# mlvlab/UP-NeRF

Measured on AMD Instinct MI355X. Metric: training rays/sec, higher is better.
Workload: dtype f32 (f16x3 emulated: 3 fp16 MFMAs per product, fp32 accumulate); 1 GPU; BASELINE.json configs[1]: Brandenburg Gate shape, 4096 rays/GPU/step, 64 coarse + 128 fine samples, two 8x256 fields + candidate/colour heads + TransientNet + appearance/candidate embeddings (763 images), pose optimisation ON, full step incl. both Adam updates; rays_per_gpu=4096, n_images=763, N_samples=64, N_importance=128, parallelism=dp1, field=f16x3

## Files before the change

upnerf_amd/csrc/common.cuh:

```cuda
#pragma once
#include <hip/hip_runtime.h>
#include <stdint.h>
#include "upnerf_hip.h"

typedef float f32x16 __attribute__((ext_vector_type(16)));
typedef float f32x4 __attribute__((ext_vector_type(4)));

#define NTHREADS 256

#define HIP_TRY(expr)                        \
  do {                                       \
    hipError_t _e = (expr);                  \
    if (_e != hipSuccess) return (int)_e;    \
  } while (0)

__device__ __forceinline__ int swz(int row, int k, int ldw) {
  return row * ldw + ((((k >> 2) ^ (row & 15)) << 2) | (k & 3));
}
__device__ __forceinline__ int swz4(int row, int k, int ldw) { return row * ldw + (((k >> 2) ^ (row & 15)) << 2); }

__device__ __forceinline__ float softplus_f(float x) { return x > 20.0f ? x : log1pf(expf(x)); }
__device__ __forceinline__ float sigmoid_f(float x) { return 1.0f / (1.0f + expf(-x)); }

__device__ __forceinline__ double wave_sum_f64(double v) {
// ... 155 lines not shown
      }
    }
  return ((unsigned long long)hi << 32) | lo;
}

template <int MT, int NT>
__device__ __forceinline__ void acc_apply_mask(f32x16 (&acc)[MT][NT], unsigned long long bits) {
  const unsigned int lo = (unsigned int)bits, hi = (unsigned int)(bits >> 32);
#pragma unroll
  for (int mt = 0; mt < MT; ++mt)
#pragma unroll
    for (int nt = 0; nt < NT; ++nt)
#pragma unroll
      for (int r = 0; r < 16; ++r) {
        const int e = (mt * NT + nt) * 16 + r;
        const bool on = e < 32 ? (lo >> e) & 1u : (hi >> (e - 32)) & 1u;
        acc[mt][nt][r] = on ? acc[mt][nt][r] : 0.0f;
      }
}

template <int MT, int NT>
__device__ __forceinline__ void acc_track_max(const f32x16 (&acc)[MT][NT], float* __restrict__ slot, int lane) {
  if (!slot) return;
  float m = 0.0f;
#pragma unroll
  for (int mt = 0; mt < MT; ++mt)
#pragma unroll
    for (int nt = 0; nt < NT; ++nt)
#pragma unroll
      for (int r = 0; r < 16; ++r) m = fmaxf(m, fabsf(acc[mt][nt][r]));
#pragma unroll
  for (int d = 32; d >= 1; d >>= 1) m = fmaxf(m, __shfl_xor(m, d));
  if (lane == 0) atomicMax((unsigned int*)slot, __float_as_uint(m));
}
__device__ __forceinline__ void wave_track_max(float m, float* __restrict__ slot, int lane) {
  if (!slot) return;
#pragma unroll
  for (int d = 32; d >= 1; d >>= 1) m = fmaxf(m, __shfl_xor(m, d));
  if (lane == 0) atomicMax((unsigned int*)slot, __float_as_uint(m));
}

template <int MT, int NT>
__device__ __forceinline__ void acc_to_lds(const f32x16 (&acc)[MT][NT], float* Hs, int ldw, int row0, int n0, int c0,
                                           int lane) {
  const int i = lane & 31, hh = lane >> 5;
#pragma unroll
  for (int mt = 0; mt < MT; ++mt)
#pragma unroll
    for (int nt = 0; nt < NT; ++nt)
#pragma unroll
      for (int r = 0; r < 16; ++r) {
        const int row = row0 + 32 * mt + (r & 3) + 8 * (r >> 2) + 4 * hh;
        Hs[swz(row, c0 + n0 + 32 * nt + i, ldw)] = acc[mt][nt][r];
      }
}

template <int TILE>
__device__ __forceinline__ void tile_store(const float* Hs, int ldw, int c0, int ncols, float* __restrict__ dst, int ldg,
                                           int m0, int M, int tid) {
  const int gpr = ncols >> 2;
  for (int idx = tid; idx < TILE * gpr; idx += NTHREADS) {
    const int row = idx / gpr, g = idx - row * gpr;
    if (m0 + row < M) {
      const f32x4 v = *(const f32x4*)&Hs[swz4(row, c0 + 4 * g, ldw)];
      *(f32x4*)&dst[(size_t)(m0 + row) * ldg + 4 * g] = v;
    }
  }
}

template <int TILE>
__device__ __forceinline__ void tile_mask_store(float* Hs, int ldw, int c0, int ncols, const float* __restrict__ act,
                                                float* __restrict__ gz, int ldg, int m0, int M, int tid) {
  const int gpr = ncols >> 2;
  for (int idx = tid; idx < TILE * gpr; idx += NTHREADS) {
    const int row = idx / gpr, g = idx - row * gpr;
    float* p = &Hs[swz4(row, c0 + 4 * g, ldw)];
    f32x4 v = {0.f, 0.f, 0.f, 0.f};
    if (m0 + row < M) {
      const size_t off = (size_t)(m0 + row) * ldg + 4 * g;
      const f32x4 av = *(const f32x4*)&act[off];
      v = *(const f32x4*)p;
      v.x = av.x > 0.f ? v.x : 0.f;
      v.y = av.y > 0.f ? v.y : 0.f;
      v.z = av.z > 0.f ? v.z : 0.f;
      v.w = av.w > 0.f ? v.w : 0.f;
      *(f32x4*)&gz[off] = v;
    }
    *(f32x4*)p = v;
  }
}

template <int TILE>
__device__ __forceinline__ void tile_rank1_store(float* Hs, int ldw, int ncols, const float* __restrict__ wrow,
                                                 const float* __restrict__ grow, int S, float* __restrict__ gz,
                                                 int m0, int M, int tid, float* __restrict__ maxslot = nullptr) {
  const int gpr = ncols >> 2;
  float lmax = 0.0f;
  for (int idx = tid; idx < TILE * gpr; idx += NTHREADS) {
    const int row = idx / gpr, g = idx - row * gpr, m = m0 + row;
    float* p = &Hs[swz4(row, 4 * g, ldw)];
    f32x4 v = {0.f, 0.f, 0.f, 0.f};
    if (m < M) {
      v = *(const f32x4*)p;
      if (grow) {
        const float w = wrow[m];
        const f32x4 gv = *(const f32x4*)&grow[(size_t)(m / S) * ncols + 4 * g];
        v.x += w * gv.x; v.y += w * gv.y; v.z += w * gv.z; v.w += w * gv.w;
      }
      *(f32x4*)&gz[(size_t)m * ncols + 4 * g] = v;
    }
    *(f32x4*)p = v;
    lmax = fmaxf(lmax, fmaxf(fmaxf(fabsf(v.x), fabsf(v.y)), fmaxf(fabsf(v.z), fabsf(v.w))));
  }
  wave_track_max(lmax, maxslot, tid & 63);
}

#define PI_F 3.14159274101257324f

__device__ __forceinline__ float mul_then_add(float o, float d, float z) {
#pragma clang fp contract(off)
  const float p = d * z;
  return o + p;
}

__device__ __forceinline__ void sincos_f32_via_f64(float arg, float& sn, float& cs) {
  const double x = (double)arg;
  const double q = rint(x * 0.63661977236758134308);
  double r = fma(-q, 1.57079632679489655800e+00, x);
  r = fma(-q, 6.12323399573676603587e-17, r);
  const double z = r * r;
  const double ps = -1.66666666666666324348e-01 + z * (8.33333333332248946124e-03 + z * (-1.98412698298579493134e-04 +
                    z * (2.75573137070700676789e-06 + z * (-2.50507602534068634195e-08 + z * 1.58969099521155010221e-10))));
  const double pc = 4.16666666666666019037e-02 + z * (-1.38888888888741095749e-03 + z * (2.48015872894767294178e-05 +
                    z * (-2.75573143513906633035e-07 + z * (2.08757232129817482790e-09 + z * -1.13596475577881948265e-11))));
  const double s = r + r * z * ps;
  const double c = 1.0 - 0.5 * z + z * z * pc;
  const int n = (int)(long long)q & 3;
  const double so = (n & 1) ? c : s, co = (n & 1) ? s : c;
  sn = (float)((n & 2) ? -so : so);
  cs = (float)(((n + 1) & 2) ? -co : co);
}

__device__ __forceinline__ float wave_sum(float v) {
#pragma unroll
  for (int d = 32; d >= 1; d >>= 1) v += __shfl_xor(v, d);
  return v;
}

#define NT_LOAD(p) __builtin_nontemporal_load(p)
#define NT_STORE(p, v) __builtin_nontemporal_store((v), (p))

#define RED_RG 8
#define RED_THREADS (64 * RED_RG)
template <int PW = RED_RG>
__device__ __forceinline__ void wgrad_reduce_body(int bid, int tid, const upnerf_wgrad_pending& P, f32x4 (*part)[64]) {
  static_assert(PW == 8 || PW == 4, "8 thread groups on 8 or 4 waves");
  const int N = P.N, K = P.K, TN = P.TN, TK = P.TK, nsplit = P.nsplit;
  const float* __restrict__ slabs = P.slabs;
  const float* __restrict__ bslabs = P.bslabs;
  const int lane = tid & 63;
  const int q = bid * 64 + lane;
  const int K4 = K >> 2;
  const int gy = (N + TN - 1) / TN, gz = (K + TK - 1) / TK;
  const bool ok = q < N * K4;
  const int n = ok ? q / K4 : 0, k = ok ? (q - n * K4) * 4 : 0;
  const int by = n / TN, bz = k / TK;
  const size_t off = ((size_t)by * gz + bz) * TN * TK + (size_t)(n - by * TN) * TK + (k - bz * TK);
  const size_t stride = (size_t)gy * gz * TN * TK;
#pragma unroll 1
  for (int rg = tid >> 6; rg < RED_RG; rg += PW) {
    f32x4 s[8];
#pragma unroll
    for (int u = 0; u < 8; ++u) s[u] = f32x4{0.f, 0.f, 0.f, 0.f};
    if (ok) {
      int sp = rg;
      for (; sp + 7 * RED_RG < nsplit; sp += 8 * RED_RG) {
        f32x4 v[8];
#pragma unroll
        for (int u = 0; u < 8; ++u) v[u] = *(const f32x4*)&slabs[off + (size_t)(sp + u * RED_RG) * stride];
#pragma unroll
        for (int u = 0; u < 8; ++u) s[u] += v[u];
      }
      for (; sp < nsplit; sp += RED_RG) s[0] += *(const f32x4*)&slabs[off + (size_t)sp * stride];
    }
    part[rg][lane] = ((s[0] + s[1]) + (s[2] + s[3])) + ((s[4] + s[5]) + (s[6] + s[7]));
  }
  __syncthreads();
  if ((tid >> 6) == 0 && ok) {
    const f32x4 t = ((part[0][lane] + part[1][lane]) + (part[2][lane] + part[3][lane])) +
                    ((part[4][lane] + part[5][lane]) + (part[6][lane] + part[7][lane]));
    if (P.n2 > 0 && n >= P.n2) *(f32x4*)&P.dW2[(size_t)(n - P.n2) * P.ldo2 + k] = t;
    else *(f32x4*)&P.dW[(size_t)n * P.ldo + k] = t;
  }
  if (P.db || (P.n2 > 0 && P.db2)) {
#pragma unroll 1
    for (int idx = bid * RED_THREADS + tid; idx < (bid + 1) * RED_THREADS; idx += 64 * PW)
    if (idx < N) {
      const int bby = idx / TN;
      float p[8] = {0.f, 0.f, 0.f, 0.f, 0.f, 0.f, 0.f, 0.f};
      const float* src = bslabs + (size_t)bby * TN + (idx - bby * TN);
      const size_t bst = (size_t)gy * TN;
      int sp = 0;
      for (; sp + 8 <= nsplit; sp += 8) {
#pragma unroll
        for (int u = 0; u < 8; ++u) p[u] += src[(size_t)(sp + u) * bst];
      }
      for (; sp < nsplit; ++sp) p[0] += src[(size_t)sp * bst];
      const float sb = ((p[0] + p[1]) + (p[2] + p[3])) + ((p[4] + p[5]) + (p[6] + p[7]));
      if (P.n2 > 0 && idx >= P.n2) { if (P.db2) P.db2[idx - P.n2] = sb; }
      else if (P.db) P.db[idx] = sb;
    }
  }
  if (P.vslabs && bid == 0) {
    for (int idx = tid; idx <= K; idx += 64 * PW) {
      float p[8] = {0.f, 0.f, 0.f, 0.f, 0.f, 0.f, 0.f, 0.f};
      const float* src = P.vslabs + idx;
      const size_t st = (size_t)K + 4;
      int sp = 0;
      for (; sp + 8 <= nsplit; sp += 8) {
#pragma unroll
        for (int u = 0; u < 8; ++u) p[u] += src[(size_t)(sp + u) * st];
      }
      for (; sp < nsplit; ++sp) p[0] += src[(size_t)sp * st];
      const float sv = ((p[0] + p[1]) + (p[2] + p[3])) + ((p[4] + p[5]) + (p[6] + p[7]));
      if (idx < K) P.dv[idx] = sv;
      else if (P.dbv) P.dbv[0] = sv;
    }
  }
}
```

upnerf_amd/csrc/wgrad_f16x3.hip:

```cpp
#include "common.cuh"
#include "wgrad_host.h"

namespace {

typedef _Float16 h8 __attribute__((ext_vector_type(8)));
typedef _Float16 h4 __attribute__((ext_vector_type(4)));
typedef short s4 __attribute__((ext_vector_type(4)));
typedef unsigned int u32x2_t __attribute__((ext_vector_type(2)));

#ifndef FX_CHUNK_BIG
#define FX_CHUNK_BIG 16
#endif

template <int FX_CHUNK>
__device__ __forceinline__ int himg(int row, int col) {
  const int panel = col >> 7, c = col & 127;
  return panel * (FX_CHUNK * 256) + 256 * row + 16 * ((c >> 3) ^ (((row & 3) << 2) | ((row >> 2) & 3))) + 2 * (c & 7);
}

__device__ __forceinline__ h4 tr_read(const char* base, int byteoff) {
  s4 v = __builtin_amdgcn_ds_read_tr16_b64_v4i16((s4 __attribute__((address_space(3)))*)(base + byteoff));
  return __builtin_bit_cast(h4, v);
}

#define FX_THREADS 512
#define WG_LOAD(p) NT_LOAD(p)
#define WG_OPLOAD(dst, p) dst = WG_LOAD((const f32x4*)(p))
#define WG_PIN_LOADS_P __builtin_amdgcn_sched_barrier(0)
template <int NP, int MTW, int NTW, bool HASV = false>
__global__ __launch_bounds__(FX_THREADS, 1) void wgrad_f16x3_kernel(int M, int N, int K, const float* __restrict__ A, int lda,
                                                                  const float* __restrict__ B, int ldb,
                                                                  const int* __restrict__ expo_a, const int* __restrict__ expo_b,
                                                                  float* __restrict__ slabs, float* __restrict__ bslabs,
                                                                  int rows_per_split, upnerf_wgrad_pending prev,
                                                                  const float* __restrict__ vrow = nullptr,
                                                                  float* __restrict__ vslabs = nullptr) {
  constexpr int TN = 64 * MTW, TK = 64 * NTW;
  constexpr int FX_CHUNK = (MTW * NTW == 16) ? FX_CHUNK_BIG : 32;
  constexpr int PN = (TN + 127) / 128, PK = (TK + 127) / 128;
  constexpr int SZA = PN * FX_CHUNK * 256, SZB = PK * FX_CHUNK * 256;
  constexpr int A4 = FX_CHUNK * TN / 4 / FX_THREADS, B4 = FX_CHUNK * TK / 4 / FX_THREADS;
  static_assert(A4 >= 1 && B4 >= 1, "tile too small for 512 threads");
  constexpr int WK = (TK >= 128) ? 4 : 2, WN = 8 / WK;
  constexpr int MT = (TN / WN >= 32) ? TN / WN / 32 : 1, NT = TK / WK / 32;
  constexpr bool HALF = TN / WN < 32;
  __shared__ __attribute__((aligned(16))) char lds[2 * (2 * SZA + 2 * SZB)];
  const int tid = threadIdx.x, lane = tid & 63, wave = tid >> 6;
  const int li = lane & 31, hh = lane >> 5;
  const bool active = !HALF || wave < 4;
  const int wn = HALF ? ((wave & 3) >> 1) : wave / WK, wk = HALF ? (wave & 1) : wave % WK;
  const int n0 = wn * 32 * MT, k0 = wk * 32 * NT;
  const int split = blockIdx.x;
  const int nblk = blockIdx.y * TN, kblk = blockIdx.z * TK;
  const int mbeg = split * rows_per_split;
  const int mend = (mbeg + rows_per_split < M) ? mbeg + rows_per_split : M;
  if (prev.nsplit > 0) {
    const int wg = (blockIdx.z * gridDim.y + blockIdx.y) * gridDim.x + blockIdx.x;
    if (wg < prev.rblocks) {
      wgrad_reduce_body(wg, tid, prev, (f32x4(*)[64])lds);
      __syncthreads();
    }
  }
  const int ea = expo_a[0], eb = expo_b[0];
  const float sa = ldexpf(1.0f, ea), sb = ldexpf(1.0f, eb);

  f32x16 acc[MT][NT];
  acc_zero(acc);
  f32x4 bsum = {0.f, 0.f, 0.f, 0.f};

  f32x4 ra0[A4], rb0[B4], ra1[A4], rb1[B4];
  float rv0[B4], rv1[B4];
  f32x4 vsum = {0.f, 0.f, 0.f, 0.f};
  float vtot = 0.0f;
  const int mlast = mend > mbeg ? mend - 1 : (mbeg < M ? mbeg : M - 1);
  auto gload = [&](f32x4 (&ra)[A4], f32x4 (&rb)[B4], float (&rv)[B4], int mc) {
#pragma unroll
    for (int q = 0; q < A4; ++q) {
      const int idx = tid + q * FX_THREADS, row = idx / (TN / 4), c4 = idx - row * (TN / 4);
      const int m = mc + row < mlast ? mc + row : mlast;
      const int col = nblk + 4 * c4 < N ? nblk + 4 * c4 : 0;
      WG_OPLOAD(ra[q], &A[(size_t)m * lda + col]);
    }
#pragma unroll
    for (int q = 0; q < B4; ++q) {
      const int idx = tid + q * FX_THREADS, row = idx / (TK / 4), c4 = idx - row * (TK / 4);
      const int m = mc + row < mlast ? mc + row : mlast;
      const int col = kblk + 4 * c4 < K ? kblk + 4 * c4 : 0;
      WG_OPLOAD(rb[q], &B[(size_t)m * ldb + col]);
      if constexpr (HASV) rv[q] = vrow[m];
    }
  };
  auto split_store = [&](char* hi, char* lo, f32x4 v, float s, int row, int col) {
    typedef float f2 __attribute__((ext_vector_type(2)));
    typedef _Float16 hh2 __attribute__((ext_vector_type(2)));
    const f2 x0 = f2{v[0], v[1]} * s, x1 = f2{v[2], v[3]} * s;
    const hh2 h0 = __builtin_convertvector(x0, hh2), h1 = __builtin_convertvector(x1, hh2);
    const int off = himg<FX_CHUNK>(row, col);
    *(h4*)(hi + off) = __builtin_shufflevector(h0, h1, 0, 1, 2, 3);
    if constexpr (NP == 2) {
      const hh2 l0 = __builtin_convertvector(x0 - __builtin_convertvector(h0, f2), hh2);
      const hh2 l1 = __builtin_convertvector(x1 - __builtin_convertvector(h1, f2), hh2);
      *(h4*)(lo + off) = __builtin_shufflevector(l0, l1, 0, 1, 2, 3);
    }
  };
  auto lstore = [&](const f32x4 (&ra)[A4], const f32x4 (&rb)[B4], const float (&rv)[B4], int buf, int mc) {
    char* base = lds + buf * (2 * SZA + 2 * SZB);
    const f32x4 z4 = {0.f, 0.f, 0.f, 0.f};
#pragma unroll
    for (int q = 0; q < A4; ++q) {
      const int idx = tid + q * FX_THREADS, row = idx / (TN / 4), c4 = idx - row * (TN / 4);
      const f32x4 v = (mc + row < mend && nblk + 4 * c4 < N) ? ra[q] : z4;
      bsum += v;
      split_store(base, base + SZA, v, sa, row, 4 * c4);
    }
#pragma unroll
    for (int q = 0; q < B4; ++q) {
      const int idx = tid + q * FX_THREADS, row = idx / (TK / 4), c4 = idx - row * (TK / 4);
      const f32x4 v = (mc + row < mend && kblk + 4 * c4 < K) ? rb[q] : z4;
      split_store(base + 2 * SZA, base + 2 * SZA + SZB, v, sb, row, 4 * c4);
      if constexpr (HASV) {
        const float vm = mc + row < mend ? rv[q] : 0.0f;
        vsum += v * vm;
        vtot += c4 == 0 ? vm : 0.0f;
      }
    }
  };
  const int g = lane >> 4, tq = (lane >> 2) & 3, tp = lane & 3;
  const int trow = 8 * (g >> 1) + tq, tcol = 16 * (g & 1) + 4 * tp;

  auto contract = [&](int buf) {
    if (!active) return;
    const char* base = lds + buf * (2 * SZA + 2 * SZB);
#pragma unroll
    for (int kk = 0; kk < FX_CHUNK / 16; ++kk) {
      h8 ah[MT], al[MT];
#pragma unroll
      for (int mt = 0; mt < MT; ++mt) {
        const int o0 = himg<FX_CHUNK>(16 * kk + trow, n0 + 32 * mt + tcol), o1 = himg<FX_CHUNK>(16 * kk + trow + 4, n0 + 32 * mt + tcol);
        const h4 x0 = tr_read(base, o0), x1 = tr_read(base, o1);
        ah[mt] = __builtin_shufflevector(x0, x1, 0, 1, 2, 3, 4, 5, 6, 7);
        if constexpr (NP == 2) {
          const h4 y0 = tr_read(base + SZA, o0), y1 = tr_read(base + SZA, o1);
          al[mt] = __builtin_shufflevector(y0, y1, 0, 1, 2, 3, 4, 5, 6, 7);
        }
      }
#pragma unroll
      for (int nt = 0; nt < NT; ++nt) {
        const int o0 = himg<FX_CHUNK>(16 * kk + trow, k0 + 32 * nt + tcol), o1 = himg<FX_CHUNK>(16 * kk + trow + 4, k0 + 32 * nt + tcol);
        const h4 x0 = tr_read(base + 2 * SZA, o0), x1 = tr_read(base + 2 * SZA, o1);
        const h8 bh = __builtin_shufflevector(x0, x1, 0, 1, 2, 3, 4, 5, 6, 7);
        h8 bl;
        if constexpr (NP == 2) {
          const h4 y0 = tr_read(base + 2 * SZA + SZB, o0), y1 = tr_read(base + 2 * SZA + SZB, o1);
          bl = __builtin_shufflevector(y0, y1, 0, 1, 2, 3, 4, 5, 6, 7);
        }
#pragma unroll
        for (int mt = 0; mt < MT; ++mt) {
          acc[mt][nt] = __builtin_amdgcn_mfma_f32_32x32x16_f16(ah[mt], bh, acc[mt][nt], 0, 0, 0);
          if constexpr (NP == 2) {
            acc[mt][nt] = __builtin_amdgcn_mfma_f32_32x32x16_f16(ah[mt], bl, acc[mt][nt], 0, 0, 0);
            acc[mt][nt] = __builtin_amdgcn_mfma_f32_32x32x16_f16(al[mt], bh, acc[mt][nt], 0, 0, 0);
          }
        }
      }
    }
  };
  constexpr bool TWO_SETS = MT * NT * 16 <= 64 || FX_CHUNK == 16;
  if constexpr (TWO_SETS) {
    gload(ra0, rb0, rv0, mbeg);
    gload(ra1, rb1, rv1, mbeg + FX_CHUNK);
#pragma unroll 1
    for (int mc = mbeg; mc < mend; mc += 2 * FX_CHUNK) {
      lstore(ra0, rb0, rv0, 0, mc);
      __syncthreads();
      gload(ra0, rb0, rv0, mc + 2 * FX_CHUNK);
      contract(0);
      lstore(ra1, rb1, rv1, 1, mc + FX_CHUNK);
      __syncthreads();
      gload(ra1, rb1, rv1, mc + 3 * FX_CHUNK);
      contract(1);
    }
  } else {
    int buf = 0;
    gload(ra0, rb0, rv0, mbeg);
#pragma unroll 1
    for (int mc = mbeg; mc < mend; mc += FX_CHUNK) {
      lstore(ra0, rb0, rv0, buf, mc);
      __syncthreads();
      gload(ra0, rb0, rv0, mc + FX_CHUNK);
      contract(buf);
      buf ^= 1;
    }
  }
  const float unscale = ldexpf(1.0f, -(ea + eb));
  const size_t blk = ((size_t)split * gridDim.y + blockIdx.y) * gridDim.z + blockIdx.z;
  float* slab = slabs + blk * TN * TK;
  if (active) {
#pragma unroll
    for (int mt = 0; mt < MT; ++mt)
#pragma unroll
      for (int nt = 0; nt < NT; ++nt)
#pragma unroll
        for (int r = 0; r < 16; ++r) {
          const int n = n0 + 32 * mt + (r & 3) + 8 * (r >> 2) + 4 * hh;
          slab[n * TK + k0 + 32 * nt + li] = acc[mt][nt][r] * unscale;
        }
  }
  if (bslabs && blockIdx.z == 0) {
    __syncthreads();
    f32x4* red = (f32x4*)lds;
    red[tid] = bsum;
    __syncthreads();
    constexpr int Q = TN / 4, G = FX_THREADS / Q;
    if (tid < Q) {
      f32x4 s = red[tid];
#pragma unroll
      for (int j = 1; j < G; ++j) s += red[tid + j * Q];
      *(f32x4*)&bslabs[((size_t)split * gridDim.y + blockIdx.y) * TN + 4 * tid] = s;
    }
  }
  if constexpr (HASV) {
    static_assert(TN == 256 && TK == 256, "the vector head rides on the 256 x 256 block");
    __syncthreads();
    f32x4* red = (f32x4*)lds;
    float* redt = (float*)(red + FX_THREADS);
    red[tid] = vsum;
    redt[tid] = vtot;
    __syncthreads();
    constexpr int Q = TK / 4, G = FX_THREADS / Q;
    if (tid < Q) {
      f32x4 s = red[tid];
#pragma unroll
      for (int j = 1; j < G; ++j) s += red[tid + j * Q];
      *(f32x4*)&vslabs[(size_t)split * (TK + 4) + 4 * tid] = s;
    }
    if (tid == 0) {
      float t = redt[0];
#pragma unroll
      for (int j = 1; j < G; ++j) t += redt[j * Q];
      vslabs[(size_t)split * (TK + 4) + TK] = t;
    }
  }
}

template <int MTW, int NTW, int PKB, int FRAG, int NP, bool HASV = false>
__global__ __launch_bounds__(FX_THREADS, 1) void wgrad_f16p_kernel(int M, int N, int K, const uint16_t* __restrict__ A, int lda,
                                                                 const int* __restrict__ aexp, const void* __restrict__ Bv, int ldb,
                                                                 const int* __restrict__ bexp, const int* __restrict__ expo_a,
                                                                 const int* __restrict__ expo_b, float* __restrict__ slabs,
                                                                 float* __restrict__ bslabs, int rows_per_split,
                                                                 upnerf_wgrad_pending prev, const uint8_t* __restrict__ Alo,
                                                                 const uint8_t* __restrict__ Blo, const float* __restrict__ vrow = nullptr,
                                                                 float* __restrict__ vslabs = nullptr) {
  static_assert(!HASV || (FRAG && PKB && NP == 1 && MTW == 4 && NTW == 4), "the vector head rides on fragment-ordered 256 x 256 problems");
  constexpr int TN = 64 * MTW, TK = 64 * NTW;
  constexpr int FX_CHUNK = (MTW * NTW == 16) ? FX_CHUNK_BIG : 32;
  constexpr int PN = (TN + 127) / 128, PK = (TK + 127) / 128;
  constexpr int SZA = PN * FX_CHUNK * 256, SZB = PK * FX_CHUNK * 256;
  constexpr int A8 = FX_CHUNK * TN / 8 / FX_THREADS;
  constexpr int B8 = PKB ? FX_CHUNK * TK / 8 / FX_THREADS : 0;
  constexpr int B4 = PKB ? 0 : FX_CHUNK * TK / 4 / FX_THREADS;
  static_assert(A8 >= 1 && (B8 >= 1 || B4 >= 1), "tile too small for 512 threads");
  constexpr int WK = (TK >= 128) ? 4 : 2, WN = 8 / WK;
  constexpr int MT = (TN / WN >= 32) ? TN / WN / 32 : 1, NT = TK / WK / 32;
  static_assert(TN / WN >= 32, "packed variant is built for 256-row blocks");
  static_assert(!FRAG || ((TN == 256 || TN == 128) && (!PKB || TK == TN) && FX_CHUNK % 16 == 0), "fragment-ordered operands are 256 or 128 wide");
  constexpr int RPA = FX_THREADS / (TN / 8), RPB = PKB ? FX_THREADS / (TK / 8) : 1;
  static_assert(!FRAG || (FX_CHUNK % RPA == 0 && (!PKB || FX_CHUNK % RPB == 0)), "whole passes per chunk");
  static_assert(NP == 1 || !FRAG, "hi + lo8 operands are row-major");
  constexpr int BUF = NP * (SZA + SZB);
  constexpr int OB = NP * SZA;
  __shared__ __attribute__((aligned(16))) char lds[2 * BUF];
  const int tid = threadIdx.x, lane = tid & 63, wave = tid >> 6;
  const int li = lane & 31, hh = lane >> 5;
  const int wn = wave / WK, wk = wave % WK;
  const int n0 = wn * 32 * MT, k0 = wk * 32 * NT;
  const int split = blockIdx.x;
  const int nblk = blockIdx.y * TN, kblk = blockIdx.z * TK;
  const int mbeg = split * rows_per_split;
  const int mend = (mbeg + rows_per_split < M) ? mbeg + rows_per_split : M;
  if (prev.nsplit > 0) {
    const int wg = (blockIdx.z * gridDim.y + blockIdx.y) * gridDim.x + blockIdx.x;
    if (wg < prev.rblocks) {
      wgrad_reduce_body(wg, tid, prev, (f32x4(*)[64])lds);
      __syncthreads();
    }
  }
  const int ea = expo_a[0], eb = expo_b[0];
  const float* __restrict__ Bf = (const float*)Bv;
  const uint16_t* __restrict__ Bh = (const uint16_t*)Bv;

  f32x16 acc[MT][NT];
  acc_zero(acc);
  float bsum[8] = {0.f, 0.f, 0.f, 0.f, 0.f, 0.f, 0.f, 0.f};

#ifndef WG_P_SETS
#define WG_P_SETS 4
#endif
  constexpr int NS = (NP == 1 && !HASV) ? WG_P_SETS : 2;
  static_assert(NS % 2 == 0, "the LDS image is double buffered: set u goes to buffer u & 1");
  h8 ra[NS][A8], rbp[NS][B8 ? B8 : 1];
  f32x4 rbf[NS][B4 ? B4 : 1];
  int xa[NS][A8], xb[NS][B8 ? B8 : 1];
  float rvv[NS][B8 ? B8 : 1];
  float vsum[8] = {0.f, 0.f, 0.f, 0.f, 0.f, 0.f, 0.f, 0.f}, vtot = 0.0f;
  u32x2_t la[NS][A8], lb[NS][B8 ? B8 : 1];
  const h8 zero8 = {0, 0, 0, 0, 0, 0, 0, 0};
  const u32x2_t mid8 = {0x80808080u, 0x80808080u};
  const int mlast = mend > mbeg ? mend - 1 : (mbeg < M ? mbeg : M - 1);
  auto gload = [&](h8 (&ra)[A8], int (&xa)[A8], h8 (&rbp)[B8 ? B8 : 1], int (&xb)[B8 ? B8 : 1], f32x4 (&rbf)[B4 ? B4 : 1],
                   u32x2_t (&la)[A8], u32x2_t (&lb)[B8 ? B8 : 1], float (&rv)[B8 ? B8 : 1], int mc) {
#pragma unroll
    for (int q = 0; q < A8; ++q) {
      if constexpr (FRAG) {
        const int mr = mc + (tid % RPA) + RPA * q, m = mr < mlast ? mr : mlast, s2 = tid / RPA;
        ra[q] = NT_LOAD((const h8*)((const char*)A + (((size_t)(m >> 5) * (TN / 16) + (s2 >> 1)) * 64 + (s2 & 1) * 32 + (m & 31)) * 16));
        xa[q] = aexp[m >> 5];
      } else {
        const int idx = tid + q * FX_THREADS, row = idx / (TN / 8), c8 = idx - row * (TN / 8);
        const int m = mc + row < mlast ? mc + row : mlast;
        const int col = nblk + 8 * c8 < N ? nblk + 8 * c8 : 0;
        ra[q] = NT_LOAD((const h8*)&A[(size_t)m * lda + col]);
        if constexpr (NP == 2) la[q] = NT_LOAD((const u32x2_t*)&Alo[(size_t)m * lda + col]);
        xa[q] = aexp[m >> 6];
      }
    }
    if constexpr (PKB) {
#pragma unroll
      for (int q = 0; q < B8; ++q) {
        if constexpr (FRAG) {
          const int mr = mc + (tid % RPB) + RPB * q, m = mr < mlast ? mr : mlast, s2 = tid / RPB;
          rbp[q] = NT_LOAD((const h8*)((const char*)Bh + (((size_t)(m >> 5) * (TK / 16) + (s2 >> 1)) * 64 + (s2 & 1) * 32 + (m & 31)) * 16));
          xb[q] = bexp[m >> 5];
          if constexpr (HASV) rv[q] = vrow[m];
        } else {
          const int idx = tid + q * FX_THREADS, row = idx / (TK / 8), c8 = idx - row * (TK / 8);
          const int m = mc + row < mlast ? mc + row : mlast;
          const int col = kblk + 8 * c8 < K ? kblk + 8 * c8 : 0;
          rbp[q] = NT_LOAD((const h8*)&Bh[(size_t)m * ldb + col]);
          if constexpr (NP == 2) lb[q] = NT_LOAD((const u32x2_t*)&Blo[(size_t)m * ldb + col]);
          xb[q] = bexp[m >> 6];
        }
      }
    } else {
#pragma unroll
      for (int q = 0; q < B4; ++q) {
        const int idx = tid + q * FX_THREADS, row = idx / (TK / 4), c4 = idx - row * (TK / 4);
        const int m = mc + row < mlast ? mc + row : mlast;
        const int col = kblk + 4 * c4 < K ? kblk + 4 * c4 : 0;
        rbf[q] = NT_LOAD((const f32x4*)&Bf[(size_t)m * ldb + col]);
      }
    }
  };
  auto scale8 = [](h8 v, int e) {
    if (e >= -24) {
      const _Float16 f = (_Float16)ldexpf(1.0f, e > 15 ? 15 : e);
#pragma unroll
      for (int j = 0; j < 8; ++j) v[j] = v[j] * f;
    } else {
      const float g = ldexpf(1.0f, e < -64 ? -64 : e);
#pragma unroll
      for (int j = 0; j < 8; ++j) v[j] = (_Float16)((float)v[j] * g);
    }
    return v;
  };
  auto lo8 = [](u32x2_t w) {
    typedef unsigned short us8 __attribute__((ext_vector_type(8)));
    us8 u;
#pragma unroll
    for (int j = 0; j < 8; ++j) u[j] = (unsigned short)((w[j >> 2] >> (8 * (j & 3))) & 0xffu);
    h8 v = __builtin_convertvector(u, h8);
#pragma unroll
    for (int j = 0; j < 8; ++j) v[j] = v[j] * (_Float16)0.03125f + (_Float16)-4.0f;
    return v;
  };
  auto lstore = [&](const h8 (&ra_)[A8], const int (&xa)[A8], const h8 (&rbp_)[B8 ? B8 : 1], const int (&xb)[B8 ? B8 : 1],
                    const f32x4 (&rbf_)[B4 ? B4 : 1], const u32x2_t (&la_)[A8], const u32x2_t (&lb_)[B8 ? B8 : 1],
                    const float (&rv)[B8 ? B8 : 1], int buf, int mc) {
    char* base = lds + buf * BUF;
    h8 ra[A8], rbp[B8 ? B8 : 1];
    f32x4 rbf[B4 ? B4 : 1];
    u32x2_t la[A8], lb[B8 ? B8 : 1];
#pragma unroll
    for (int q = 0; q < A8; ++q) {
      const int idx = tid + q * FX_THREADS;
      const bool ok = FRAG ? (mc + (tid % RPA) + RPA * q < mend) : (mc + idx / (TN / 8) < mend && nblk + 8 * (idx % (TN / 8)) < N);
      ra[q] = ok ? ra_[q] : zero8;
      la[q] = ok ? la_[q] : mid8;
    }
#pragma unroll
    for (int q = 0; q < B8; ++q) {
      const int idx = tid + q * FX_THREADS;
      const bool ok = FRAG ? (mc + (tid % RPB) + RPB * q < mend) : (mc + idx / (TK / 8) < mend && kblk + 8 * (idx % (TK / 8)) < K);
      rbp[q] = ok ? rbp_[q] : zero8;
      lb[q] = ok ? lb_[q] : mid8;
    }
#pragma unroll
    for (int q = 0; q < B4; ++q) {
      const int idx = tid + q * FX_THREADS;
      rbf[q] = (mc + idx / (TK / 4) < mend && kblk + 4 * (idx % (TK / 4)) < K) ? rbf_[q] : f32x4{0.f, 0.f, 0.f, 0.f};
    }
#pragma unroll
    for (int q = 0; q < A8; ++q) {
      const int idx = tid + q * FX_THREADS, row = idx / (TN / 8), c8 = idx - row * (TN / 8);
      const float inv = ldexpf(1.0f, -xa[q]);
#pragma unroll
      for (int j = 0; j < 8; ++j) bsum[j] += (float)ra[q][j] * inv;
      const h8 v = scale8(ra[q], ea - xa[q]);
      if constexpr (NP == 2) {
        const h8 vl = lo8(la[q]);
#pragma unroll
        for (int j = 0; j < 8; ++j) bsum[j] += (float)vl[j] * inv;
        *(h8*)(base + SZA + himg<FX_CHUNK>(row, 8 * c8)) = scale8(vl, ea - xa[q]);
      }
      if constexpr (FRAG) {
        const int r = (tid % RPA) + RPA * q, s2 = tid / RPA, col = 16 * (s2 >> 1) + 4 * (s2 & 1);
        *(h4*)(base + himg<FX_CHUNK>(r, col)) = __builtin_shufflevector(v, v, 0, 1, 2, 3);
        *(h4*)(base + himg<FX_CHUNK>(r, col + 8)) = __builtin_shufflevector(v, v, 4, 5, 6, 7);
      } else {
        *(h8*)(base + himg<FX_CHUNK>(row, 8 * c8)) = v;
      }
    }
    if constexpr (PKB) {
#pragma unroll
      for (int q = 0; q < B8; ++q) {
        const int idx = tid + q * FX_THREADS, row = idx / (TK / 8), c8 = idx - row * (TK / 8);
        h8 v = rbp[q];
        if constexpr (HASV) {
          const bool in = mc + (tid % RPB) + RPB * q < mend;
          const float sc = in ? ldexpf(rv[q], -xb[q]) : 0.0f;
#pragma unroll
          for (int j = 0; j < 8; ++j) vsum[j] = fmaf((float)v[j], sc, vsum[j]);
          vtot += (in && tid < RPB) ? rv[q] : 0.0f;
        }
        v = scale8(v, eb - xb[q]);
        if constexpr (FRAG) {
          const int r = (tid % RPB) + RPB * q, s2 = tid / RPB, col = 16 * (s2 >> 1) + 4 * (s2 & 1);
          *(h4*)(base + OB + himg<FX_CHUNK>(r, col)) = __builtin_shufflevector(v, v, 0, 1, 2, 3);
          *(h4*)(base + OB + himg<FX_CHUNK>(r, col + 8)) = __builtin_shufflevector(v, v, 4, 5, 6, 7);
        } else {
          *(h8*)(base + OB + himg<FX_CHUNK>(row, 8 * c8)) = v;
          if constexpr (NP == 2) *(h8*)(base + OB + SZB + himg<FX_CHUNK>(row, 8 * c8)) = scale8(lo8(lb[q]), eb - xb[q]);
        }
      }
    } else {
      const float sb = ldexpf(1.0f, eb);
#pragma unroll
      for (int q = 0; q < B4; ++q) {
        const int idx = tid + q * FX_THREADS, row = idx / (TK / 4), c4 = idx - row * (TK / 4);
        typedef float f2 __attribute__((ext_vector_type(2)));
        typedef _Float16 hh2 __attribute__((ext_vector_type(2)));
        const f2 x0 = f2{rbf[q][0], rbf[q][1]} * sb, x1 = f2{rbf[q][2], rbf[q][3]} * sb;
        const hh2 h0 = __builtin_convertvector(x0, hh2), h1 = __builtin_convertvector(x1, hh2);
        *(h4*)(base + OB + himg<FX_CHUNK>(row, 4 * c4)) = __builtin_shufflevector(h0, h1, 0, 1, 2, 3);
        if constexpr (NP == 2) {
          const hh2 l0 = __builtin_convertvector(x0 - __builtin_convertvector(h0, f2), hh2);
          const hh2 l1 = __builtin_convertvector(x1 - __builtin_convertvector(h1, f2), hh2);
          *(h4*)(base + OB + SZB + himg<FX_CHUNK>(row, 4 * c4)) = __builtin_shufflevector(l0, l1, 0, 1, 2, 3);
        }
      }
    }
  };
  const int g = lane >> 4, tq = (lane >> 2) & 3, tp = lane & 3;
  const int trow = 8 * (g >> 1) + tq, tcol = 16 * (g & 1) + 4 * tp;
  auto contract = [&](int buf) {
    const char* base = lds + buf * BUF;
#pragma unroll
    for (int kk = 0; kk < FX_CHUNK / 16; ++kk) {
      h8 ah[MT], al[MT];
#pragma unroll
      for (int mt = 0; mt < MT; ++mt) {
        const int o0 = himg<FX_CHUNK>(16 * kk + trow, n0 + 32 * mt + tcol), o1 = himg<FX_CHUNK>(16 * kk + trow + 4, n0 + 32 * mt + tcol);
        const h4 x0 = tr_read(base, o0), x1 = tr_read(base, o1);
        ah[mt] = __builtin_shufflevector(x0, x1, 0, 1, 2, 3, 4, 5, 6, 7);
        if constexpr (NP == 2) {
          const h4 y0 = tr_read(base + SZA, o0), y1 = tr_read(base + SZA, o1);
          al[mt] = __builtin_shufflevector(y0, y1, 0, 1, 2, 3, 4, 5, 6, 7);
        }
      }
#pragma unroll
      for (int nt = 0; nt < NT; ++nt) {
        const int o0 = himg<FX_CHUNK>(16 * kk + trow, k0 + 32 * nt + tcol), o1 = himg<FX_CHUNK>(16 * kk + trow + 4, k0 + 32 * nt + tcol);
        const h4 x0 = tr_read(base + OB, o0), x1 = tr_read(base + OB, o1);
        const h8 bh = __builtin_shufflevector(x0, x1, 0, 1, 2, 3, 4, 5, 6, 7);
        h8 bl;
        if constexpr (NP == 2) {
          const h4 y0 = tr_read(base + OB + SZB, o0), y1 = tr_read(base + OB + SZB, o1);
          bl = __builtin_shufflevector(y0, y1, 0, 1, 2, 3, 4, 5, 6, 7);
        }
#pragma unroll
        for (int mt = 0; mt < MT; ++mt) {
          acc[mt][nt] = __builtin_amdgcn_mfma_f32_32x32x16_f16(ah[mt], bh, acc[mt][nt], 0, 0, 0);
          if constexpr (NP == 2) {
            acc[mt][nt] = __builtin_amdgcn_mfma_f32_32x32x16_f16(ah[mt], bl, acc[mt][nt], 0, 0, 0);
            acc[mt][nt] = __builtin_amdgcn_mfma_f32_32x32x16_f16(al[mt], bh, acc[mt][nt], 0, 0, 0);
          }
        }
      }
    }
  };
#pragma unroll
  for (int u = 0; u < NS; ++u) {
    gload(ra[u], xa[u], rbp[u], xb[u], rbf[u], la[u], lb[u], rvv[u], mbeg + u * FX_CHUNK);
    WG_PIN_LOADS_P;
  }
#pragma unroll 1
  for (int mc = mbeg; mc < mend; mc += NS * FX_CHUNK) {
#pragma unroll
    for (int u = 0; u < NS; ++u) {
      lstore(ra[u], xa[u], rbp[u], xb[u], rbf[u], la[u], lb[u], rvv[u], u & 1, mc + u * FX_CHUNK);
      __syncthreads();
      gload(ra[u], xa[u], rbp[u], xb[u], rbf[u], la[u], lb[u], rvv[u], mc + (NS + u) * FX_CHUNK);
      WG_PIN_LOADS_P;
      contract(u & 1);
    }
  }
  const float unscale = ldexpf(1.0f, -(ea + eb));
  const size_t blk = ((size_t)split * gridDim.y + blockIdx.y) * gridDim.z + blockIdx.z;
  float* slab = slabs + blk * TN * TK;
#pragma unroll
  for (int mt = 0; mt < MT; ++mt)
#pragma unroll
    for (int nt = 0; nt < NT; ++nt)
#pragma unroll
      for (int r = 0; r < 16; ++r) {
        const int n = n0 + 32 * mt + (r & 3) + 8 * (r >> 2) + 4 * hh;
        slab[n * TK + k0 + 32 * nt + li] = acc[mt][nt][r] * unscale;
      }
  if (bslabs && blockIdx.z == 0) {
    __syncthreads();
    float* red = (float*)lds;
#pragma unroll
    for (int j = 0; j < 8; ++j) red[tid * 8 + j] = bsum[j];
    __syncthreads();
    constexpr int Q = TN / 8, G = FX_THREADS / Q;
    if (tid < TN) {
      float sacc = 0.0f;
      if constexpr (FRAG) {
        const int s2 = 2 * (tid >> 4) + ((tid >> 2) & 1), j = 4 * ((tid >> 3) & 1) + (tid & 3);
#pragma unroll
        for (int t = 0; t < RPA; ++t) sacc += red[(s2 * RPA + t) * 8 + j];
      } else {
        const int grp = tid >> 3, j = tid & 7;
#pragma unroll
        for (int t = 0; t < G; ++t) sacc += red[(grp + t * Q) * 8 + j];
      }
      bslabs[((size_t)split * gridDim.y + blockIdx.y) * TN + tid] = sacc;
    }
  }
  if constexpr (HASV) {
    __syncthreads();
    float* red = (float*)lds;
    float* redt = red + 8 * FX_THREADS;
#pragma unroll
    for (int j = 0; j < 8; ++j) red[tid * 8 + j] = vsum[j];
    if (tid < RPB) redt[tid] = vtot;
    __syncthreads();
    if (tid < TK) {
      const int s2 = 2 * (tid >> 4) + ((tid >> 2) & 1), j = 4 * ((tid >> 3) & 1) + (tid & 3);
      float sacc = 0.0f;
#pragma unroll
      for (int t = 0; t < RPB; ++t) sacc += red[(s2 * RPB + t) * 8 + j];
      vslabs[(size_t)split * (TK + 4) + tid] = sacc;
    }
    if (tid == 0) {
      float t = 0.0f;
#pragma unroll
      for (int r = 0; r < RPB; ++r) t += redt[r];
      vslabs[(size_t)split * (TK + 4) + TK] = t;
    }
  }
}


#define WP_CH 16
#define WP_SLOTS 5
#define WP_SLOT (4 * 8192)
__global__ __launch_bounds__(FX_THREADS, 1) void wgrad_planes_kernel(int M, const uint16_t* __restrict__ Ah, const uint16_t* __restrict__ Al,
                                                                   const int* __restrict__ aexp, const uint16_t* __restrict__ Bh,
                                                                   const uint16_t* __restrict__ Bl, const int* __restrict__ bexp,
                                                                   const int* __restrict__ expo_a, const int* __restrict__ expo_b,
                                                                   float* __restrict__ slabs, float* __restrict__ bslabs,
                                                                   int rows_per_split, upnerf_wgrad_pending prev) {
  constexpr int TN = 256, TK = 256, MT = 4, NT = 2, SZ = 8192;
  __shared__ __attribute__((aligned(16))) char lds[WP_SLOTS * WP_SLOT];
  const int tid = threadIdx.x, lane = tid & 63, wave = __builtin_amdgcn_readfirstlane(tid >> 6);
  const int li = lane & 31, hh = lane >> 5;
  const int wn = wave >> 2, wk = wave & 3;
  const int n0 = wn * 32 * MT, k0 = wk * 32 * NT;
  const int split = blockIdx.x;
  const int mbeg = split * rows_per_split;
  const int mend = (mbeg + rows_per_split < M) ? mbeg + rows_per_split : M;
  if (prev.nsplit > 0) {
    if ((int)blockIdx.x < prev.rblocks) {
      wgrad_reduce_body(blockIdx.x, tid, prev, (f32x4(*)[64])lds);
      __syncthreads();
    }
  }
  const int ea = expo_a[0], eb = expo_b[0];
  f32x16 acc[MT][NT];
  acc_zero(acc);
  float bacc = 0.0f;
  const int nchunk = mend > mbeg ? (mend - mbeg) / WP_CH : 0;
  const int p = wave >> 1, panel = wave & 1;
  const char* __restrict__ src = (const char*)(p == 0 ? Ah : (p == 1 ? Al : (p == 2 ? Bh : Bl)));
  int soff[4];
#pragma unroll
  for (int rg = 0; rg < 4; ++rg) {
    const int row = 4 * rg + (lane >> 4), pos = lane & 15;
    soff[rg] = row * 512 + panel * 256 + ((pos ^ (((row & 3) << 2) | (row >> 2))) << 4);
  }
  auto dma_piece = [&](int c, int rg) {
    const int cc = c < nchunk ? c : nchunk - 1;
    const char* a = src + (size_t)(mbeg + cc * WP_CH) * 512 + soff[rg];
    const unsigned d = (unsigned)(size_t)((__attribute__((address_space(3))) char*)lds) + (c % WP_SLOTS) * WP_SLOT + p * SZ + panel * 4096;
    asm volatile("s_mov_b32 m0, %0\n\ts_nop 0\n\tglobal_load_lds_dwordx4 %1, off nt" ::"s"(d + rg * 1024), "v"(a) : "memory", "m0");
  };
  auto dma = [&](int c) {
    const int cc = c < nchunk ? c : nchunk - 1;
    const char* g = src + (size_t)(mbeg + cc * WP_CH) * 512;
    const unsigned d = (unsigned)(size_t)((__attribute__((address_space(3))) char*)lds) + (c % WP_SLOTS) * WP_SLOT + p * SZ + panel * 4096;
#pragma unroll
    for (int rg = 0; rg < 4; ++rg) {
      const char* a = g + soff[rg];
      asm volatile("s_mov_b32 m0, %0\n\ts_nop 0\n\tglobal_load_lds_dwordx4 %1, off nt" ::"s"(d + rg * 1024), "v"(a) : "memory", "m0");
    }
  };
  const int g4 = lane >> 4, tq = (lane >> 2) & 3, tp = lane & 3;
  const int trow = 8 * (g4 >> 1) + tq, tcol = 16 * (g4 & 1) + 4 * tp;
  if (nchunk > 0) {
    __syncthreads();
    dma(0);
    dma(1);
    dma(2);
    dma(3);
    int nxa = aexp[mbeg >> 6], nxb = bexp[mbeg >> 6];
#pragma unroll 1
    for (int c = 0; c < nchunk; ++c) {
      const int xa = nxa, xb = nxb;
      asm volatile("s_waitcnt vmcnt(12)" ::: "memory");
      __builtin_amdgcn_s_waitcnt(0xC07F);
      __builtin_amdgcn_s_barrier();
      asm volatile("" ::: "memory");
      dma(c + 4);
      {
        const int mn = mbeg + (c + 1 < nchunk ? c + 1 : c) * WP_CH;
        nxa = aexp[mn >> 6];
        nxb = bexp[mn >> 6];
      }
      const char* base = lds + (c % WP_SLOTS) * WP_SLOT;
      const int fa = ea - xa, fb = eb - xb;
      auto scale8 = [](h8 v, int e) {
        if (e >= -24) {
          const _Float16 f = (_Float16)ldexpf(1.0f, e > 15 ? 15 : e);
#pragma unroll
          for (int j = 0; j < 8; ++j) v[j] = v[j] * f;
        } else {
          const float g = ldexpf(1.0f, e < -64 ? -64 : e);
// ... 216 lines not shown
```

Before: 257,000 rays/s.

## Overlap deferred wgrad reduction with first operand loads; parallelize bias/v reductions

In both wgrad kernels, the first global operand loads are now issued before the fused reduction of the previous layer's split-K slabs. Their latency can then hide behind the reduction work instead of following it. The bias and v-vector reductions in the reduce body now give each output eight lanes that sum strided splits and combine them with shuffles. These reductions are spread across all reduce blocks (v in reverse block order) instead of one thread per output and only block 0 for v. This keeps more registers live during the reduction and may change float summation order.

```diff
diff --git a/upnerf_amd/csrc/common.cuh b/upnerf_amd/csrc/common.cuh
--- a/upnerf_amd/csrc/common.cuh
+++ b/upnerf_amd/csrc/common.cuh
@@ -331,6 +331,25 @@
 
 #define RED_RG 8
 #define RED_THREADS (64 * RED_RG)
+__device__ __forceinline__ float wgrad_sum8(const float* __restrict__ src, size_t stride, int nsplit, int u) {
+  const int full = nsplit & ~7;
+  float p = 0.0f;
+  int sp = u;
+  for (; sp + 56 < full; sp += 64) {
+    float v[8];
+#pragma unroll
+    for (int j = 0; j < 8; ++j) v[j] = src[(size_t)(sp + 8 * j) * stride];
+#pragma unroll
+    for (int j = 0; j < 8; ++j) p += v[j];
+  }
+  for (; sp < full; sp += 8) p += src[(size_t)sp * stride];
+  if (u == 0)
+    for (sp = full; sp < nsplit; ++sp) p += src[(size_t)sp * stride];
+  p += __shfl_xor(p, 1);
+  p += __shfl_xor(p, 2);
+  p += __shfl_xor(p, 4);
+  return p;
+}
 template <int PW = RED_RG>
 __device__ __forceinline__ void wgrad_reduce_body(int bid, int tid, const upnerf_wgrad_pending& P, f32x4 (*part)[64]) {
   static_assert(PW == 8 || PW == 4, "8 thread groups on 8 or 4 waves");
@@ -373,37 +392,27 @@
   }
   if (P.db || (P.n2 > 0 && P.db2)) {
 #pragma unroll 1
-    for (int idx = bid * RED_THREADS + tid; idx < (bid + 1) * RED_THREADS; idx += 64 * PW)
-    if (idx < N) {
-      const int bby = idx / TN;
-      float p[8] = {0.f, 0.f, 0.f, 0.f, 0.f, 0.f, 0.f, 0.f};
-      const float* src = bslabs + (size_t)bby * TN + (idx - bby * TN);
-      const size_t bst = (size_t)gy * TN;
-      int sp = 0;
-      for (; sp + 8 <= nsplit; sp += 8) {
-#pragma unroll
-        for (int u = 0; u < 8; ++u) p[u] += src[(size_t)(sp + u) * bst];
-      }
-      for (; sp < nsplit; ++sp) p[0] += src[(size_t)sp * bst];
-      const float sb = ((p[0] + p[1]) + (p[2] + p[3])) + ((p[4] + p[5]) + (p[6] + p[7]));
-      if (P.n2 > 0 && idx >= P.n2) { if (P.db2) P.db2[idx - P.n2] = sb; }
-      else if (P.db) P.db[idx] = sb;
-    }
-  }
-  if (P.vslabs && bid == 0) {
-    for (int idx = tid; idx <= K; idx += 64 * PW) {
-      float p[8] = {0.f, 0.f, 0.f, 0.f, 0.f, 0.f, 0.f, 0.f};
-      const float* src = P.vslabs + idx;
-      const size_t st = (size_t)K + 4;
-      int sp = 0;
-      for (; sp + 8 <= nsplit; sp += 8) {
-#pragma unroll
-        for (int u = 0; u < 8; ++u) p[u] += src[(size_t)(sp + u) * st];
-      }
-      for (; sp < nsplit; ++sp) p[0] += src[(size_t)sp * st];
-      const float sv = ((p[0] + p[1]) + (p[2] + p[3])) + ((p[4] + p[5]) + (p[6] + p[7]));
-      if (idx < K) P.dv[idx] = sv;
-      else if (P.dbv) P.dbv[0] = sv;
-    }
-  }
-}
+    for (int base = bid * 8 * PW; base < N; base += P.rblocks * 8 * PW) {
+      const int idx = base + (tid >> 3);
+      const bool in = idx < N;
+      const int bby = in ? idx / TN : 0;
+      const float sb = wgrad_sum8(bslabs + (in ? (size_t)bby * TN + (idx - bby * TN) : 0), (size_t)gy * TN, nsplit, tid & 7);
+      if (in && (tid & 7) == 0) {
+        if (P.n2 > 0 && idx >= P.n2) { if (P.db2) P.db2[idx - P.n2] = sb; }
+        else if (P.db) P.db[idx] = sb;
+      }
+    }
+  }
+  if (P.vslabs) {
+#pragma unroll 1
+    for (int base = (P.rblocks - 1 - bid) * 8 * PW; base <= K; base += P.rblocks * 8 * PW) {
+      const int idx = base + (tid >> 3);
+      const bool in = idx <= K;
+      const float sv = wgrad_sum8(P.vslabs + (in ? idx : 0), (size_t)K + 4, nsplit, tid & 7);
+      if (in && (tid & 7) == 0) {
+        if (idx < K) P.dv[idx] = sv;
+        else if (P.dbv) P.dbv[0] = sv;
+      }
+    }
+  }
+}
diff --git a/upnerf_amd/csrc/wgrad_f16x3.hip b/upnerf_amd/csrc/wgrad_f16x3.hip
--- a/upnerf_amd/csrc/wgrad_f16x3.hip
+++ b/upnerf_amd/csrc/wgrad_f16x3.hip
@@ -54,19 +54,8 @@
   const int nblk = blockIdx.y * TN, kblk = blockIdx.z * TK;
   const int mbeg = split * rows_per_split;
   const int mend = (mbeg + rows_per_split < M) ? mbeg + rows_per_split : M;
-  if (prev.nsplit > 0) {
-    const int wg = (blockIdx.z * gridDim.y + blockIdx.y) * gridDim.x + blockIdx.x;
-    if (wg < prev.rblocks) {
-      wgrad_reduce_body(wg, tid, prev, (f32x4(*)[64])lds);
-      __syncthreads();
-    }
-  }
   const int ea = expo_a[0], eb = expo_b[0];
   const float sa = ldexpf(1.0f, ea), sb = ldexpf(1.0f, eb);
-
-  f32x16 acc[MT][NT];
-  acc_zero(acc);
-  f32x4 bsum = {0.f, 0.f, 0.f, 0.f};
 
   f32x4 ra0[A4], rb0[B4], ra1[A4], rb1[B4];
   float rv0[B4], rv1[B4];
@@ -90,6 +79,19 @@
       if constexpr (HASV) rv[q] = vrow[m];
     }
   };
+  constexpr bool TWO_SETS = MT * NT * 16 <= 64 || FX_CHUNK == 16;
+  gload(ra0, rb0, rv0, mbeg);
+  if constexpr (TWO_SETS) gload(ra1, rb1, rv1, mbeg + FX_CHUNK);
+  if (prev.nsplit > 0) {
+    const int wg = (blockIdx.z * gridDim.y + blockIdx.y) * gridDim.x + blockIdx.x;
+    if (wg < prev.rblocks) {
+      wgrad_reduce_body(wg, tid, prev, (f32x4(*)[64])lds);
+      __syncthreads();
+    }
+  }
+  f32x16 acc[MT][NT];
+  acc_zero(acc);
+  f32x4 bsum = {0.f, 0.f, 0.f, 0.f};
   auto split_store = [&](char* hi, char* lo, f32x4 v, float s, int row, int col) {
     typedef float f2 __attribute__((ext_vector_type(2)));
     typedef _Float16 hh2 __attribute__((ext_vector_type(2)));
@@ -165,10 +167,7 @@
       }
     }
   };
-  constexpr bool TWO_SETS = MT * NT * 16 <= 64 || FX_CHUNK == 16;
   if constexpr (TWO_SETS) {
-    gload(ra0, rb0, rv0, mbeg);
-    gload(ra1, rb1, rv1, mbeg + FX_CHUNK);
 #pragma unroll 1
     for (int mc = mbeg; mc < mend; mc += 2 * FX_CHUNK) {
       lstore(ra0, rb0, rv0, 0, mc);
@@ -182,7 +181,6 @@
     }
   } else {
     int buf = 0;
-    gload(ra0, rb0, rv0, mbeg);
 #pragma unroll 1
     for (int mc = mbeg; mc < mend; mc += FX_CHUNK) {
       lstore(ra0, rb0, rv0, buf, mc);
@@ -279,19 +277,11 @@
   const int nblk = blockIdx.y * TN, kblk = blockIdx.z * TK;
   const int mbeg = split * rows_per_split;
   const int mend = (mbeg + rows_per_split < M) ? mbeg + rows_per_split : M;
-  if (prev.nsplit > 0) {
-    const int wg = (blockIdx.z * gridDim.y + blockIdx.y) * gridDim.x + blockIdx.x;
-    if (wg < prev.rblocks) {
-      wgrad_reduce_body(wg, tid, prev, (f32x4(*)[64])lds);
-      __syncthreads();
-    }
-  }
   const int ea = expo_a[0], eb = expo_b[0];
   const float* __restrict__ Bf = (const float*)Bv;
   const uint16_t* __restrict__ Bh = (const uint16_t*)Bv;
 
   f32x16 acc[MT][NT];
-  acc_zero(acc);
   float bsum[8] = {0.f, 0.f, 0.f, 0.f, 0.f, 0.f, 0.f, 0.f};
 
 #ifndef WG_P_SETS
@@ -504,6 +494,14 @@
     gload(ra[u], xa[u], rbp[u], xb[u], rbf[u], la[u], lb[u], rvv[u], mbeg + u * FX_CHUNK);
     WG_PIN_LOADS_P;
   }
+  if (prev.nsplit > 0) {
+    const int wg = (blockIdx.z * gridDim.y + blockIdx.y) * gridDim.x + blockIdx.x;
+    if (wg < prev.rblocks) {
+      wgrad_reduce_body(wg, tid, prev, (f32x4(*)[64])lds);
+      __syncthreads();
+    }
+  }
+  acc_zero(acc);
 #pragma unroll 1
   for (int mc = mbeg; mc < mend; mc += NS * FX_CHUNK) {
 #pragma unroll
```

Measured after the change: 259,300 rays/s, median of 6. About the same (+0.9%).
